# evandez/neuron-descriptions

Hardware: AMD Instinct MI355X
Metric: neuron-descriptions/sec (whole node), 4096 neurons x k=15 exemplars (higher is better)
Workload: dtype f32-equivalent: operands split into (hi,lo) f16 pairs (22 significant bits), 3 f16 MFMAs per product, f32 accumulate

## Files before the change

### neuron-descriptions_amd/csrc/common.h

```cpp
#pragma once
#include <hip/hip_runtime.h>
#include <stdint.h>
#include <stddef.h>
#include <string>
#include <vector>
#include <map>

#include "../../include/milan_hip.h"

#ifndef MILAN_EXPERIMENTS
#define MILAN_EXPERIMENTS 0
#endif

namespace milan {

void set_error(const char* fmt, ...);
#define MILAN_CHECK_HIP(expr)                                              \
  do {                                                                     \
    hipError_t _e = (expr);                                                \
    if (_e != hipSuccess) {                                                \
      milan::set_error("%s:%d: %s -> %s", __FILE__, __LINE__, #expr,       \
                       hipGetErrorString(_e));                             \
      return (int)_e;                                                      \
    }                                                                      \
// ... 54 lines not shown
  int chunk_major;
  float* C2;
  float* Cs;
  unsigned* status;
  int f16;
  const float* Wt;
  int tap_inner;
  const long long* lse_tgt;
  long lse_tgt_stride;
  float* lse_x;
  const int* m_live;
  const int* row_list;
  int m_live_mul;
  int tap_ncls;
  int tap_cls[MILAN_TAP_CLASSES][5];
};
static_assert(sizeof(GemmArgs) % 4 == 0, "GemmArgs is reloaded word by word");

enum OutMode : int { OUT_SCALAR = 0, OUT_VEC4 = 1, OUT_SPLIT8 = 2, OUT_F16 = 3 };

int launch_gemm(const GemmArgs& g, hipStream_t s);
bool row_list_supported(const GemmArgs& g);
void set_status_word(unsigned* word);
unsigned* status_word();
void profile_tag_kernel(int family);
int launch_zero_fill(void* p, size_t bytes, hipStream_t s);
int launch_f32_to_split(const float* src, long ld_src, float* dst, long ld_dst,
                        long rows, int K, float scale, hipStream_t s, int* nanrow = nullptr,
                        int stamp = 0);
int gemm_profile_enable(int enable);
int ensure_lds_attr(const void* kern, int bytes);
int device_cus8(int* out);
// ... 415 lines not shown
```

### neuron-descriptions_amd/csrc/decoder.hip

```cpp
#include "common.h"
#include <limits>
#include <optional>

namespace milan {

static constexpr float kFloatMin = -3.402823466e+38f;

static const Tensor* find(milan_ctx* c, const std::string& name) {
  auto it = c->raw.find(name);
  return it == c->raw.end() ? nullptr : &it->second;
}

__global__ void pack_rows_kernel(const float* __restrict__ src, int n, int k,
                                 int kp, float* __restrict__ dst) {
  const long total = (long)n * kp;
  for (long idx = blockIdx.x * (long)blockDim.x + threadIdx.x; idx < total;
       idx += (long)gridDim.x * blockDim.x) {
    const int r = idx / kp, col = idx - (long)r * kp;
    dst[idx] = col < k ? src[(long)r * k + col] : 0.f;
  }
}

__device__ inline int lstm_source_row(int i, int hidden) {
  if (!hidden) return i;
// ... 1722 lines not shown
  if (j < *live) out[j] = seqs[(long)urow[j] * L + col];
}

__global__ void lm_gather_rows_kernel(const float4* __restrict__ src, const int* __restrict__ idx,
                                      const int* __restrict__ live, int w4,
                                      float4* __restrict__ dst) {
  const long total = (long)*live * w4;
  for (long i = blockIdx.x * (long)blockDim.x + threadIdx.x; i < total;
       i += (long)gridDim.x * blockDim.x) {
    const long j = i / w4;
    const int q = (int)(i - j * w4);
    dst[i] = src[(long)idx[j] * w4 + q];
  }
}

struct LmDedup {
  int *cls, *urow, *par, *U;
  float *gh, *gc, *gv;
  int64_t *tok_c, *tgt_c;
};

static size_t lm_dedup_floats(const milan_dims& d, size_t R, int L, int G) {
  const size_t maps = 5 * (size_t)(L + 1) * R + 2 * (size_t)(L + 1) * G + (size_t)(L + 1) + 64;
  const size_t state = (2 * (size_t)d.lm_layers + 1) * R * d.lm_hidden_size;
  return maps + state + 4 * R + 2048;
}

static int lm_score_dedup(milan_ctx* c, const int64_t* seqs, int rows, int L, int group,
                          const int32_t* seq_len, int len_div, float* total, DecBuf* b,
                          float* scratch, hipStream_t s) {
// ... 11 lines not shown
  q.cls = (int*)take(sizeof(int) * (size_t)(L + 1) * R);
  q.urow = (int*)take(sizeof(int) * (size_t)(L + 1) * R);
  q.par = (int*)take(sizeof(int) * (size_t)(L + 1) * R);
  q.U = (int*)take(sizeof(int) * (size_t)(L + 1));
  q.gh = (float*)take(sizeof(float) * (size_t)d.lm_layers * R * Hl);
  q.gc = (float*)take(sizeof(float) * (size_t)d.lm_layers * R * Hl);
  q.gv = (float*)take(sizeof(float) * (size_t)R * Hl);
  q.tok_c = (int64_t*)take(sizeof(int64_t) * (size_t)R);
  q.tgt_c = (int64_t*)take(sizeof(int64_t) * (size_t)R);
  hipLaunchKernelGGL(lm_prefix_classes_kernel, dim3(G), dim3(256), 0, s, seqs, L, group, R, G,
                     rep, lrank, cnt);
  hipLaunchKernelGGL(lm_prefix_scan_kernel, dim3(L + 1), dim3(256), 0, s, cnt, G, offs, q.U);
  hipLaunchKernelGGL(lm_prefix_assign_kernel, dim3(nblk_all(R)), dim3(256), 0, s, rep, lrank, offs,
                     L, group, R, G, q.cls, q.urow, q.par);
  MILAN_CHECK_HIP(hipGetLastError());
  const size_t st_floats = (size_t)d.lm_layers * R * Hl;
  MILAN_TRY(launch_zero_fill(q.gh, sizeof(float) * st_floats, s));
  MILAN_TRY(launch_zero_fill(q.gc, sizeof(float) * st_floats, s));
  float* hs = b->lm_gates;
  float* emb_s = c->scratch;
  const size_t layer_sz = (size_t)R * Hl;
  int cur = 0;
  for (int t = 0; t + 1 < L; ++t) {
    const int p1 = t + 1, p2 = t + 2;
    const int* U1 = q.U + p1;
    const int* U2 = q.U + p2;
    LmState& st = b->lm[cur];
    LmState& nx = b->lm[cur ^ 1];
    hipLaunchKernelGGL(lm_gather_tok_kernel, dim3(nblk_all(R)), dim3(256), 0, s, seqs, (long)L, t,
                       q.urow + (size_t)p1 * R, U1, q.tok_c);
    hipLaunchKernelGGL(embed_split_kernel, dim3(nblk((long)R * (El / 8))), dim3(256), 0, s,
                       c->lm_embedding, q.tok_c, R, El, emb_s, El, c->emb_scale, status_word(),
                       U1);
    if (t > 0) {
      for (int l = 0; l < d.lm_layers; ++l) {
        hipLaunchKernelGGL(lm_gather_rows_kernel, dim3(nblk((long)R * (Hl / 4), 8192)), dim3(256),
// ... 48 lines not shown
    cur ^= 1;
  }
  MILAN_CHECK_HIP(hipGetLastError());
  return 0;
}

static int lm_score_impl(milan_ctx* c, const int64_t* seqs, int rows, int L,
                         const int32_t* seq_len, int len_div, float* total,
                         DecBuf* b, hipStream_t s, int group = 1,
                         float* dedup_scratch = nullptr, size_t dedup_floats = 0) {
  const milan_dims& d = c->d;
  MILAN_REQUIRE(d.has_lm && c->lm_out.w, MILAN_ERR_NO_LM,
                "cannot use MI/rerank decoding without an LM");
  const size_t st_bytes =
      sizeof(float) * (size_t)b->lm[0].rows * d.lm_hidden_size * d.lm_layers;
  MILAN_TRY(launch_zero_fill(b->lm[0].h, st_bytes, s));
  MILAN_TRY(launch_zero_fill(b->lm[0].c, st_bytes, s));
  if (L < 2) {
    MILAN_TRY(launch_zero_fill(total, sizeof(float) * rows, s));
    return 0;
  }
  int cur = 0;
  const bool split = lm_split_ok(c, rows) && (long)rows == b->lm[0].rows;
  static const bool lse_on = !(getenv("MILAN_LM_LSE") && atoi(getenv("MILAN_LM_LSE")) == 0);
  const bool lse = lse_on && d.vocab_size % 4 == 0 && d.vocab_size >= 256;
  if (split)
    MILAN_TRY(launch_zero_fill(b->lm_gates, sizeof(float) * (size_t)rows * d.lm_hidden_size * d.lm_layers, s));
  static const bool dedup_on = !(getenv("MILAN_LM_DEDUP") && atoi(getenv("MILAN_LM_DEDUP")) == 0);
  if (dedup_on && split && lse && group > 1 && group <= 256 && rows % group == 0 && dedup_scratch &&
      d.lm_hidden_size % 4 == 0 &&
      lm_dedup_floats(d, (size_t)rows, L, rows / group) <= dedup_floats)
    return lm_score_dedup(c, seqs, rows, L, group, seq_len, len_div, total, b, dedup_scratch, s);
  for (int t = 0; t + 1 < L; ++t) {
    hipLaunchKernelGGL(gather_col_kernel, dim3(nblk_all(rows)), dim3(256), 0, s, seqs,
                       (long)rows, (long)L, t, b->tok);
    if (split && lse) {
      const int nb = (d.vocab_size + 63) / 64;
      MILAN_TRY(lm_step_split(c, b->tok, rows, b->lm[cur], b->lm[cur ^ 1],
                              b->lm_gates, cur, b->lm_logits, s, seqs + t + 1, (long)L));
      hipLaunchKernelGGL(lm_accumulate_lse_kernel, dim3((rows + 3) / 4), dim3(256), 0, s,
                         b->lm_logits, nb, b->lm_logits + (size_t)rows * 2 * nb, rows, seqs,
                         (long)L, t, seq_len, len_div, d.stop_index, b->lm_alive, total);
      cur ^= 1;
      continue;
    }
    if (split)
      MILAN_TRY(lm_step_split(c, b->tok, rows, b->lm[cur], b->lm[cur ^ 1],
// ... 262 lines not shown
```

### neuron-descriptions_amd/csrc/encoder.hip

```cpp
#include "common.h"
#include <optional>
#include <vector>

#include <cstdlib>

namespace milan {

static constexpr float kBnEps = 1e-5f;

__global__ void pack_conv_kernel(const float* __restrict__ w, int cout, int cin,
                                 int cinp, int kh, int kw, int kp,
                                 const float* __restrict__ gamma,
                                 const float* __restrict__ beta,
                                 const float* __restrict__ mean,
                                 const float* __restrict__ var,
                                 float* __restrict__ wp,
                                 float* __restrict__ bias) {
  const long total = (long)cout * kp;
  for (long idx = blockIdx.x * (long)blockDim.x + threadIdx.x; idx < total;
       idx += (long)gridDim.x * blockDim.x) {
    const int o = idx / kp, k = idx - (long)o * kp;
    const int tap = k / cinp, i = k - tap * cinp;
    float v = 0.f;
    if (tap < kh * kw && i < cin) {
// ... 1034 lines not shown
  Levels lv;
  int h1, w1, hp, wp;
  float *in4, *raw, *x0, *x1, *ds, *t1, *t2;
  size_t x_sz, t1_sz, t2_sz;
  int *list_idx, *list_n;
  float* list_w;
  int* bbox;
  int* poison;
  int *order, *bbox_c, *count;
  int *tail_loc, *tail_cnt, *tail_off, *tail_rows, *tail_U;
  void* sh_hash;
  int *sh_rep, *sh_flag, *class_of;
  unsigned char* tail_s0;
  int *tail_loc3, *tail_cnt3, *tail_off3, *tail_rows3, *tail_U3;
  unsigned char* tail_s3;
};

static int conv_out(int h, int k, int s, int p) { return (h + 2 * p - k) / s + 1; }

static int plan(const milan_ctx* c, int n, int H, int W, Arena& a, EncPlan* pl) {
  const int wd = c->d.trunk_width;
  pl->h1 = conv_out(H, 7, 2, 3); pl->w1 = conv_out(W, 7, 2, 3);
  pl->hp = conv_out(pl->h1, 3, 2, 1); pl->wp = conv_out(pl->w1, 3, 2, 1);
  Levels& lv = pl->lv;
  lv.h[0] = pl->h1; lv.w[0] = pl->w1;
  lv.h[1] = pl->hp; lv.w[1] = pl->wp;
  for (int l = 2; l < 5; ++l) {
    lv.h[l] = conv_out(lv.h[l - 1], 3, 2, 1);
    lv.w[l] = conv_out(lv.w[l - 1], 3, 2, 1);
  }
// ... 33 lines not shown
    pl->tail_cnt = a.get<int>(3 * (size_t)n);
    pl->tail_off = a.get<int>(3 * (size_t)n);
    pl->tail_U = a.get<int>(4);
    pl->sh_hash = a.get<unsigned long long>((size_t)n);
    pl->sh_rep = a.get<int>((size_t)n);
    pl->sh_flag = a.get<int>((size_t)n);
    pl->class_of = a.get<int>((size_t)n);
    pl->tail_s0 = a.get<unsigned char>(((size_t)n * P4 + 3) & ~(size_t)3);
    const size_t P3 = (size_t)lv.h[3] * lv.w[3];
    pl->tail_loc3 = a.get<int>(2 * (size_t)n * P3);
    pl->tail_rows3 = a.get<int>(2 * (size_t)n * P3);
    pl->tail_cnt3 = a.get<int>(2 * (size_t)n);
    pl->tail_off3 = a.get<int>(2 * (size_t)n);
    pl->tail_U3 = a.get<int>(4);
    pl->tail_s3 = a.get<unsigned char>(((size_t)n * P3 + 3) & ~(size_t)3);
  }
  return 0;
}

static int encoder_sub_batch() {
  static int v = 0;
  if (v == 0) {
    const char* e = getenv("MILAN_ENC_SUB");
    v = e ? atoi(e) : 9600;
    if (v < 1) v = 9600;
  }
  return v;
}

static void alexnet_workspace_dry(const milan_ctx* c, int n, int H, int W,
// ... 437 lines not shown
    MILAN_TRY(lin(acol, 9 * P, b.c2, b.c2.wst, t2c, P, EPI_BIAS_RELU, nullptr, UO));
    hipLaunchKernelGGL(tail_rows_kernel<false>, dim3(blocks_for(rows_all * (Cin / 4))), dim3(256), 0, s,
                       (const float4*)X, rowsO, UO, Cin / 4, (float4*)rg);
    MILAN_TRY(lin(t2c, P, b.c3, b.c3.ws, yc, Cout, EPI_BIAS_RES_RELU, rg, UO));
    hipLaunchKernelGGL(tail_rows_kernel<true>, dim3(blocks_for(rows_all * (Cout / 4))), dim3(256), 0, s,
                       (const float4*)yc, rowsO, UO, Cout / 4, (float4*)Y);
    MILAN_CHECK_HIP(hipGetLastError());
    return 0;
  };

  auto on_list = [&](GemmArgs g, const int* rows, const int* U) {
    g.row_list = rows; g.m_live = U; g.m_live_mul = 1;
    return g;
  };
  auto list_ok = [&](const GemmArgs& g) { return row_list_supported(on_list(g, pl.tail_rows, pl.tail_U)); };
  auto tail_block_args = [&](const Bottleneck& b, const float* X, float* Y, float* T1, int hh,
                             int ww, GemmArgs* g1, GemmArgs* g2, GemmArgs* g3) {
    int h1, w1, h2, w2, h3, w3;
    *g1 = conv_args(b.c1, X, n, hh, ww, T1, EPI_BIAS_RELU, nullptr, c->zero, &h1, &w1, true);
    *g2 = conv_args(b.c2, T1, n, h1, w1, pl.t2, EPI_BIAS_RELU, nullptr, c->zero, &h2, &w2, true);
    *g3 = conv_args(b.c3, pl.t2, n, h2, w2, Y, EPI_BIAS_RES_RELU, X, c->zero, &h3, &w3, true);
  };
  auto tail_block_lists_ok = [&](const Bottleneck& b, int hh, int ww) {
    GemmArgs g1, g2, g3;
    tail_block_args(b, pl.x0, pl.x1, pl.t1, hh, ww, &g1, &g2, &g3);
    return lists && list_ok(g1) && list_ok(g2) && list_ok(g3);
  };
  auto tail_block_lists = [&](const Bottleneck& b, const float* X, float* Y, float* T1, int hh,
                              int ww, int kM, int kO) -> int {
    GemmArgs g1, g2, g3;
    tail_block_args(b, X, Y, T1, hh, ww, &g1, &g2, &g3);
    const int* rowsM = pl.tail_rows + (long)kM * n * P4;
    const int* rowsO = pl.tail_rows + (long)kO * n * P4;
    MILAN_TRY(launch_gemm(on_list(g1, rowsM, pl.tail_U + kM), s));
    MILAN_TRY(launch_gemm(on_list(g2, rowsO, pl.tail_U + kO), s));
    MILAN_TRY(launch_gemm(on_list(g3, rowsO, pl.tail_U + kO), s));
    return 0;
  };
  auto two_source_args = [&](const Bottleneck& b, const float* xin, float* yo, int hh, int ww,
                             int h2, int w2, int* h3, int* w3) {
    GemmArgs g3 = conv_args(b.c3d, pl.t2, n, h2, w2, yo, EPI_BIAS_RELU,
                            nullptr, c->zero, h3, w3, true);
    g3.Cin = b.c3.cin;
    g3.a_pix_stride = b.c3.cin;
    g3.a_img_stride = (long)h2 * w2 * b.c3.cin;
    g3.A2 = xin; g3.K1 = b.c3.K; g3.H2 = hh; g3.W2d = ww;
    g3.stride2 = b.down.stride;
    g3.a2_pix_stride = b.down.cin;
    g3.a2_img_stride = (long)hh * ww * b.down.cin;
    g3.flop_k = b.c3.K + b.down.K;
// ... 175 lines not shown
                   w2 == w && chain_supported(chain_P, b.down.cin, chain_NR);
      }
      const bool conv_front =
          (chain_plain || chain_ds) && (c->fusion & MILAN_FUSE_BNECK) && b.c2.K == b.c2.Kp &&
          b.c2.bias_s && conv3_p64_supported(b.c2.cin, b.c2.cout, b.c2.kh, b.c2.kw, b.c2.stride,
                                             b.c2.pad) &&
          chain_conv_supported(chain_P, chain_ds ? b.down.cin : 0, chain_NR, h1, w1);
      const bool c1_front =
          conv_front && c1_pending && chain_ds && b.c1.ws && b.c1.bias_s && b.c1.kh == 1 &&
          b.c1.kw == 1 && b.c1.stride == 1 && b.c1.cin == 64 && b.c1.cout == 64 &&
          b.c1.K == b.c1.Kp && h1 == h && w1 == w &&
          chain_conv_c1_supported(chain_P, b.down.cin, chain_NR, h1, w1);
      if (k0 >= 0 && li == 3 && bi == 0 && !chain_plain && !chain_ds && h == h3l && w == w3l) {
        const int* rows0 = pl.tail_rows + (long)k0 * n * P4;
        if (c1_pending) MILAN_TRY(launch_gemm(on_list(g1, rowsV, pl.tail_U3), s));
        MILAN_TRY(launch_gemm(on_list(g2, rows0, pl.tail_U + k0), s));
        GemmArgs g3 = two_source_args(b, x, y, h, w, h2, w2, &h3, &w3);
        MILAN_TRY(launch_gemm(on_list(g3, rows0, pl.tail_U + k0), s));
        float* tmp = x; x = y; y = tmp;
        h = h3; w = w3;
        continue;
      }
      if (lists_l3 && k0 >= 0 && li == 2 && last_of_stage && !chain_plain && !chain_ds &&
          h == h3l && w == w3l) {
        if (c1_pending) MILAN_TRY(gemm_t(g1));
        MILAN_TRY(launch_gemm(on_list(g2, rowsW, pl.tail_U3 + 1), s));
        GemmArgs g3 = conv_args(b.c3, pl.t2, n, h2, w2, y, EPI_BIAS_RES_RELU, x, c->zero, &h3, &w3, split);
        MILAN_TRY(launch_gemm(on_list(g3, rowsW, pl.tail_U3 + 1), s));
        float* tmp = x; x = y; y = tmp;
        h = h3; w = w3;
        continue;
      }
      if (c1_pending && !c1_front) MILAN_TRY(gemm_t(g1));
      if (conv_front) {
      } else if (split && (c->fusion & MILAN_FUSE_CONV3) && b.c2.K == b.c2.Kp &&
          conv3_p64_supported(b.c2.cin, b.c2.cout, b.c2.kh, b.c2.kw, b.c2.stride,
                              b.c2.pad)) {
        Conv3Args ca{};
        ca.in = t1buf; ca.ws = b.c2.ws; ca.bias = b.c2.bias_s; ca.acc_scale = b.c2.ws_inv;
        ca.out = pl.t2; ca.zero = c->zero; ca.n = n; ca.h = h1; ca.w = w1;
        ca.n_live = live;
// ... 378 lines not shown
```

### neuron-descriptions_amd/csrc/gemm.hip

```cpp
#include "common.h"

#include <map>
#include <mutex>
#include <utility>

#include <cstdio>
#include <cstdlib>
#include <cstring>
#include <type_traits>
#include <utility>
#include <vector>

#ifndef MILAN_ABLATE_BUILD
#define MILAN_ABLATE_BUILD 0
#endif
#ifndef MILAN_EXPERIMENTS
#define MILAN_EXPERIMENTS 0
#endif

namespace milan {

typedef float f32x16 __attribute__((ext_vector_type(16)));
typedef float f32x4 __attribute__((ext_vector_type(4)));
typedef _Float16 f16x8 __attribute__((ext_vector_type(8)));
// ... 1444 lines not shown

struct PpLoader {
  __amdgpu_buffer_rsrc_t srd_a, srd_a2, srd_w, cur_srd;
  unsigned row_off[4], row_off2[4], voff[4], vb[4];
  int hw0[4];
  unsigned mask[4];
  int ia, iw, is_kh, is_kw, is_cin0, seg_soff, cin_limit;
  unsigned a_bits, w_bits;
  int w_slice;
};

struct TapTile {
  int y0, ny, x0, nx;
  unsigned mask;
  int cnt, j, tile_n;
};

__device__ __forceinline__ bool tap_tile(const GemmArgs& g, int tiles_m, int tiles_n, TapTile* t) {
  const int b = blockIdx.x;
  if (g.tap_ncls == 0) {
    const int T = tiles_m * tiles_n;
    if (b >= T) return false;
    const int tile = xcd_tile(b, T);
    t->j = tile / tiles_n;
    t->tile_n = tile - t->j * tiles_n;
    t->y0 = 0; t->ny = g.Ho; t->x0 = 0; t->nx = g.Wo;
    t->mask = 0xffffffffu >> (32 - g.KH * g.KW);
    t->cnt = g.M;
    return true;
  }
// ... 6 lines not shown
    const int T = c < g.tap_ncls ? ((imgs * cw[c * 5 + 1] * cw[c * 5 + 3] + 255) >> 8) * tiles_n : 0;
    const int B = (T + 7) & ~7;
    if (cls < 0 && b < first + B) { cls = c; cfirst = first; ctiles = T; }
    first += B;
  }
  if (cls < 0) return false;
  const int bl = b - cfirst;
  if ((bl >> 3) >= (ctiles >> 3) + ((bl & 7) < (ctiles & 7))) return false;
  const int tile = xcd_tile(bl, ctiles);
  t->j = tile / tiles_n;
  t->tile_n = tile - t->j * tiles_n;
  t->y0 = cw[cls * 5]; t->ny = cw[cls * 5 + 1]; t->x0 = cw[cls * 5 + 2]; t->nx = cw[cls * 5 + 3];
  t->mask = (unsigned)cw[cls * 5 + 4];
  t->cnt = imgs * t->ny * t->nx;
  return true;
}

template <int BNW, bool F16 = false, bool TAPI = false, bool LIST = false>
__device__ __forceinline__ void split16_pp32_tile(int tile_m, int tile_n, int tid, bool prefetched,
                                                  bool has_next, int ntile_m, int ntile_n,
                                                  TapTile tt = TapTile{}) {
  const GemmArgs g = reload_gemm_args();
  constexpr int BM = 256, BN = 256, BKP = 32, TM = BNW == 256 ? 4 : 2, TN = 2;
  static_assert(BNW == 256 || BNW == 128, "ping-pong tile: 256 or 128 columns");
  constexpr int SLOTF = BM * BKP;
  constexpr unsigned OOB = 0x80000000u;
  extern __shared__ __attribute__((aligned(16))) float smem[];
  auto a_slot = [&](int sl) { return smem + (sl < 2 ? sl : 3) * SLOTF; };
  auto w_slot = [&](int sl) { return smem + (sl == 0 ? 2 : 4) * SLOTF; };
  const int lane = tid & 63;
// ... 36 lines not shown
    else x = rem0 + (ok ? row : 0);
    int dimg = (int)((float)x * r_howo);
    dimg -= (dimg * pix_img > x);
    dimg += ((dimg + 1) * pix_img <= x);
    const int rem = x - dimg * pix_img;
    int ho = (int)((float)rem * r_wo);
    ho -= (ho * pix_row > rem);
    ho += ((ho + 1) * pix_row <= rem);
    *dimg_out = dimg;
    *wo_out = rem - ho * pix_row + (TAPI ? tt.x0 : 0);
    *ho_out = ho + (TAPI ? tt.y0 : 0);
    return ok;
  };
  auto setup = [&](PpLoader& L, int tm, int tn) {
    const int prow = lane >> 3, pos = lane & 7;
    const int m0 = tm * BM;
    const int img0 = LIST ? list_slot0(m0) : m0 / pix_img;
    const int rem0 = LIST ? img0 * pix_img : m0 - img0 * pix_img;
    const long bias = ((long)g.pad * g.Wd + g.pad) * g.a_pix_stride;
    L.srd_a = __builtin_amdgcn_make_buffer_rsrc(
        const_cast<float*>(g.A + (long)img0 * g.a_img_stride - bias), 0, 0x7fffffff, 0x00020000);
    L.srd_a2 = __builtin_amdgcn_make_buffer_rsrc(
        const_cast<float*>(g.A2 ? g.A2 + (long)img0 * g.a2_img_stride : g.A), 0, 0x7fffffff,
        0x00020000);
    L.srd_w = __builtin_amdgcn_make_buffer_rsrc(const_cast<float*>(g.W + (long)tn * BNW * g.Kp), 0,
                                                0x7fffffff, 0x00020000);
#pragma unroll
    for (int it = 0; it < 4; ++it) {
      const int row = it * 64 + wave * 8 + prow;
      const int q = pos ^ ((row >> 1) & 7);
      int dimg, ho, wo;
// ... 256 lines not shown
  __builtin_amdgcn_s_barrier();
  if (has_next) {
    PpLoader N;
    setup(N, ntile_m, ntile_n);
    issue_a(N, I0{}, true);
    issue_w(N, I0{}, true);
    issue_a(N, I1{}, true);
  }
  const GemmArgs ge = reload_gemm_args<LIST>();
#pragma unroll
  for (int i = 0; i < TM; ++i)
#pragma unroll
    for (int j = 0; j < TN; ++j) acc[i][j] = acc[i][j] * ge.acc_scale;
  if constexpr (LIST) {
    int* tab = reinterpret_cast<int*>(a_slot(0)) + wave * (TM * 32);
    const int m0 = tile_m * BM;
#pragma unroll
    for (int e = 0; e < TM * 32 / 64; ++e) {
      const int r = e * 64 + lane;
      const int m = m0 + wm * (TM * 32) + r;
      tab[r] = m < rows_all ? ge.row_list[m] : 0x7fffffff;
    }
    run_epilogue<TM, TN, true, true>(ge, acc, a_slot(2), wave, lane, 0, tile_n * BNW + wn * 64, tab);
  } else if constexpr (TAPI) {
    int* tab = reinterpret_cast<int*>(a_slot(0)) + wave * (TM * 32);
    const int m0 = tile_m * BM;
    const int img0 = m0 / pix_img;
    const int rem0 = m0 - img0 * pix_img;
#pragma unroll
    for (int e = 0; e < TM * 32 / 64; ++e) {
      const int r = e * 64 + lane;
// ... 53 lines not shown
template <int BNW>
__global__ __launch_bounds__(512, 2) void igemm_split16_pp32t_kernel(GemmArgs g, int tiles_m,
                                                                     int tiles_n) {
  tiles_m = live_tiles_m(g, tiles_m, 256);
  TapTile tt;
  if (!tap_tile(g, tiles_m, tiles_n, &tt)) return;
  int tid = threadIdx.x;
  asm volatile("" : "+v"(tid));
  split16_pp32_tile<BNW, false, true>(tt.j, tt.tile_n, tid, false, false, tt.j, tt.tile_n, tt);
}

template <bool TAPI>
__global__ __launch_bounds__(512, 2) void igemm_split16_pp32l_kernel(GemmArgs g, int tiles_m,
                                                                     int tiles_n) {
  tiles_m = live_tiles_m(g, tiles_m, 256);
  const int T = tiles_m * tiles_n;
  const int q = blockIdx.x;
  if (q >= T) return;
  const int tile = xcd_tile(q, T);
  const int tile_m = tile / tiles_n, tile_n = tile - tile_m * tiles_n;
  TapTile tt{};
  if constexpr (TAPI) {
    tt.ny = g.Ho; tt.nx = g.Wo;
    tt.mask = 0xffffffffu >> (32 - g.KH * g.KW);
    tt.cnt = g.M;
  }
  int tid = threadIdx.x;
  asm volatile("" : "+v"(tid));
  split16_pp32_tile<256, false, TAPI, true>(tile_m, tile_n, tid, false, false, tile_m, tile_n, tt);
}

template <int BNW, bool TAPI>
__global__ __launch_bounds__(512, 2) void igemm_f16_pp32_kernel(GemmArgs g, int tiles_m, int tiles_n) {
  tiles_m = live_tiles_m(g, tiles_m, 256);
  if constexpr (TAPI) {
    TapTile tt;
    if (!tap_tile(g, tiles_m, tiles_n, &tt)) return;
    int tid = threadIdx.x;
    asm volatile("" : "+v"(tid));
    split16_pp32_tile<BNW, true, true>(tt.j, tt.tile_n, tid, false, false, tt.j, tt.tile_n, tt);
// ... 500 lines not shown
  auto kern = igemm_split16_tm2_kernel<BM, BN, STAGES>;
  MILAN_TRY(ensure_lds_attr(reinterpret_cast<const void*>(kern), (int)lds));
  hipLaunchKernelGGL(kern, dim3(tiles_m * tiles_n), dim3(NT), lds, s, g, tiles_m,
                     tiles_n);
  MILAN_CHECK_HIP(hipGetLastError());
  return 0;
}

static bool tap_inner_wanted(const GemmArgs& g) {
  static int on = -1;
  if (on < 0) { const char* e = getenv("MILAN_TAP_INNER"); on = e ? atoi(e) : 1; }
  return on && g.Wt && !g.A2 && g.KH * g.KW > 1 && g.KH * g.KW <= 32 && g.K == g.Kp &&
         g.Cin % 32 == 0;
}

static int tap_classes(GemmArgs& t, int tiles_m, int tiles_n) {
  static int on = -1;
  if (on < 0) { const char* e = getenv("MILAN_TAP_SKIP"); on = e ? atoi(e) : 1; }
  const bool wanted = on && t.tap_ncls >= 0;
  t.tap_ncls = 0;
  const int howo = t.Ho * t.Wo;
  if (!wanted || howo <= 0 || t.M % howo != 0 || (t.m_live && t.m_live_mul % howo != 0))
    return tiles_m * tiles_n;
  struct Run { int o0, n; unsigned set; };
  auto runs = [](int size, int out, int k, int stride, int pad, Run* r) {
    int n = 0;
    for (int o = 0; o < out; ++o) {
      unsigned set = 0;
      for (int i = 0; i < k; ++i)
        if (o * stride - pad + i >= 0 && o * stride - pad + i < size) set |= 1u << i;
      if (n > 0 && r[n - 1].set == set) { ++r[n - 1].n; continue; }
      if (n == MILAN_TAP_CLASSES) return MILAN_TAP_CLASSES + 1;
      r[n++] = Run{o, 1, set};
    }
    return n;
  };
  Run ry[MILAN_TAP_CLASSES], rx[MILAN_TAP_CLASSES];
  const int nry = runs(t.H, t.Ho, t.KH, t.stride, t.pad, ry);
  const int nrx = runs(t.Wd, t.Wo, t.KW, t.stride, t.pad, rx);
  if (nry * nrx > MILAN_TAP_CLASSES) return tiles_m * tiles_n;
  int cls[MILAN_TAP_CLASSES][5], n = 0, min_pix = howo;
  for (int a = 0; a < nry; ++a)
    for (int b = 0; b < nrx; ++b, ++n) {
      unsigned mask = 0;
      for (int kh = 0; kh < t.KH; ++kh)
        for (int kw = 0; kw < t.KW; ++kw)
          if ((ry[a].set >> kh & 1u) && (rx[b].set >> kw & 1u)) mask |= 1u << (kh * t.KW + kw);
      if (mask == 0) return tiles_m * tiles_n;
      const int c[5] = {ry[a].o0, ry[a].n, rx[b].o0, rx[b].n, (int)mask};
      int at = n;
      while (at > 0 && __builtin_popcount((unsigned)cls[at - 1][4]) < __builtin_popcount(mask)) {
        memcpy(cls[at], cls[at - 1], sizeof(c));
        --at;
      }
      memcpy(cls[at], c, sizeof(c));
      if (ry[a].n * rx[b].n < min_pix) min_pix = ry[a].n * rx[b].n;
    }
  if ((256L / min_pix + 2) * t.a_img_stride * 4 + 64 >= 0x7fffffffL) return tiles_m * tiles_n;
  const long imgs = t.M / howo;
  long grid = 0;
  for (int c = 0; c < n; ++c)
    grid += ((imgs * cls[c][1] * cls[c][3] + 255) / 256 * tiles_n + 7) / 8 * 8;
  if (grid >= 0x7fffffffL) return tiles_m * tiles_n;
  t.tap_ncls = n;
  memcpy(t.tap_cls, cls, sizeof(int) * 5 * n);
  return (int)grid;
}

static thread_local bool t_row_list_taken = false;

template <int BNW>
static int launch_split16_pp32(const GemmArgs& g, hipStream_t s) {
  const int tiles_m = (g.M + 255) / 256, tiles_n = (g.N + BNW - 1) / BNW;
  const size_t lds = size_t(5) * 256 * 32 * sizeof(float);
  if (g.row_list != nullptr) {
    if (BNW != 256) return MILAN_ERR_SHAPE;
    t_row_list_taken = true;
    GemmArgs t = g;
    const bool tapi = tap_inner_wanted(g);
    if (tapi) { t.W = g.Wt; t.tap_inner = 1; }
    t.tap_ncls = 0;
    profile_tag_kernel(tapi ? MILAN_KERNEL_PP32T_256 : MILAN_KERNEL_PP32_256);
    auto kern = tapi ? igemm_split16_pp32l_kernel<true> : igemm_split16_pp32l_kernel<false>;
    MILAN_TRY(ensure_lds_attr(reinterpret_cast<const void*>(kern), (int)lds));
    hipLaunchKernelGGL(kern, dim3(tiles_m * tiles_n), dim3(512), lds, s, t, tiles_m, tiles_n);
    MILAN_CHECK_HIP(hipGetLastError());
    return 0;
  }
  if (tap_inner_wanted(g)) {
    GemmArgs t = g;
    t.W = g.Wt;
    t.tap_inner = 1;
    const int grid = tap_classes(t, tiles_m, tiles_n);
    profile_tag_kernel(BNW == 256 ? MILAN_KERNEL_PP32T_256 : MILAN_KERNEL_PP32_128);
    auto kern = igemm_split16_pp32t_kernel<BNW>;
    MILAN_TRY(ensure_lds_attr(reinterpret_cast<const void*>(kern), (int)lds));
    hipLaunchKernelGGL(kern, dim3(grid), dim3(512), lds, s, t, tiles_m, tiles_n);
    MILAN_CHECK_HIP(hipGetLastError());
    return 0;
  }
// ... 169 lines not shown
bool row_list_supported(const GemmArgs& g) {
  static int pp = -1;
  if (pp < 0) { const char* e = getenv("MILAN_PP"); pp = e ? atoi(e) : 1; }
  const long howo = (long)g.Ho * g.Wo;
  if (g.row_list == nullptr || g.m_live == nullptr || g.m_live_mul != 1) return false;
  if (!g.a_split || g.f16 || g.chunk_major || g.aniso || g.tile_hint != 0 || env_tile_hint() != 0 ||
      env_tile_override(g.N, g.K) != 0 || pp != 1)
    return false;
#if MILAN_EXPERIMENTS
  if (conv3x3_enabled() || (getenv("MILAN_SCHED") && atoi(getenv("MILAN_SCHED")))) return false;
#endif
  if (g.epilogue == EPI_LSE || g.epilogue == EPI_LSTM || !g.out_split) return false;
  if (g.N % 256 != 0 || g.Cin % 32 != 0 || g.K != g.Kp || !pp_eligible(g)) return false;
  if (g.A2 && (g.K1 % 32 != 0 || g.KH != 1 || g.KW != 1)) return false;
  if (g.KH * g.KW > 1 && !tap_inner_wanted(g)) return false;
  if ((long)g.H + g.pad >= 32768 || (long)g.Wd + g.pad >= 32768) return false;
  if (howo <= 0 || g.M % howo != 0 || 257 * howo >= (1L << 24)) return false;
  if (258 * g.a_img_stride * 4 + 64 >= 0x7fffffffL) return false;
  if (g.A2 && 258 * g.a2_img_stride * 4 + 64 >= 0x7fffffffL) return false;
  return true;
}

static int launch_gemm_impl(GemmArgs g, hipStream_t s) {
  const bool cin32 = (g.Cin % 32 == 0);
  if (g.status == nullptr) g.status = status_word();
  if (g.tile_hint == 0) g.tile_hint = env_tile_hint();
  if (const int o = env_tile_override(g.N, g.K)) g.tile_hint = o;
  {
    static int dbg = -1;
    if (dbg < 0) { const char* e = getenv("MILAN_ABLATE"); dbg = e ? atoi(e) : 0; }
// ... 160 lines not shown
```

Baseline: 1439.

## Sort row-list 3x3 conv rows by tap class to skip padded taps

Adds count, scan and fill kernels that regroup the sparse row list of the tail-stage 3x3 convolutions by border tap class. The row-list GEMM kernel then walks per-class segments and applies each class's tap mask, so it skips padded taps for border pixels. The LM dedup path now runs before the full-state zero fills, and a row-limited zero kernel replaces its own full zero fills. The cost is three extra small launches per sorted GEMM, more grid tiles with partial-tile waste per segment, and a serial segment search at the start of each block.

```diff
diff --git a/neuron-descriptions_amd/csrc/common.h b/neuron-descriptions_amd/csrc/common.h
--- a/neuron-descriptions_amd/csrc/common.h
+++ b/neuron-descriptions_amd/csrc/common.h
@@ -92,8 +92,29 @@
   int m_live_mul;
   int tap_ncls;
   int tap_cls[MILAN_TAP_CLASSES][5];
+  const int* list_seg;
+  int list_nseg;
 };
 static_assert(sizeof(GemmArgs) % 4 == 0, "GemmArgs is reloaded word by word");
+
+constexpr int MILAN_LIST_SEGS = 36;
+struct RowListClasses {
+  int ncls, blk_slots, nblk;
+  int cls[MILAN_TAP_CLASSES][5];
+};
+bool row_list_classes(const GemmArgs& g, RowListClasses* rc);
+inline size_t row_list_sort_ints(size_t n) { return 2 * n * MILAN_TAP_CLASSES; }
+int launch_row_list_sort(const RowListClasses& rc, const int* loc, const int* cnt, int n, int P,
+                         int Wo, int* scratch, int* seg, int* rows, hipStream_t s);
+inline GemmArgs on_sorted_list(GemmArgs g, const RowListClasses& rc, const int* rows,
+                               const int* seg, const int* live) {
+  g.row_list = rows; g.m_live = live; g.m_live_mul = 1;
+  g.list_seg = seg; g.list_nseg = rc.nblk * rc.ncls;
+  g.tap_ncls = rc.ncls;
+  for (int c = 0; c < rc.ncls; ++c)
+    for (int i = 0; i < 5; ++i) g.tap_cls[c][i] = rc.cls[c][i];
+  return g;
+}
 
 enum OutMode : int { OUT_SCALAR = 0, OUT_VEC4 = 1, OUT_SPLIT8 = 2, OUT_F16 = 3 };
 
diff --git a/neuron-descriptions_amd/csrc/decoder.hip b/neuron-descriptions_amd/csrc/decoder.hip
--- a/neuron-descriptions_amd/csrc/decoder.hip
+++ b/neuron-descriptions_amd/csrc/decoder.hip
@@ -1760,6 +1760,18 @@
   }
 }
 
+__global__ void lm_zero_rows_kernel(const int* __restrict__ live, int w4, int layers, long layer4,
+                                    float4* __restrict__ a, float4* __restrict__ b) {
+  const long total = (long)*live * w4;
+  const float4 z = make_float4(0.f, 0.f, 0.f, 0.f);
+  for (long i = blockIdx.x * (long)blockDim.x + threadIdx.x; i < total;
+       i += (long)gridDim.x * blockDim.x)
+    for (int l = 0; l < layers; ++l) {
+      a[l * layer4 + i] = z;
+      b[l * layer4 + i] = z;
+    }
+}
+
 struct LmDedup {
   int *cls, *urow, *par, *U;
   float *gh, *gc, *gv;
@@ -1801,12 +1813,12 @@
   hipLaunchKernelGGL(lm_prefix_assign_kernel, dim3(nblk_all(R)), dim3(256), 0, s, rep, lrank, offs,
                      L, group, R, G, q.cls, q.urow, q.par);
   MILAN_CHECK_HIP(hipGetLastError());
-  const size_t st_floats = (size_t)d.lm_layers * R * Hl;
-  MILAN_TRY(launch_zero_fill(q.gh, sizeof(float) * st_floats, s));
-  MILAN_TRY(launch_zero_fill(q.gc, sizeof(float) * st_floats, s));
   float* hs = b->lm_gates;
   float* emb_s = c->scratch;
   const size_t layer_sz = (size_t)R * Hl;
+  hipLaunchKernelGGL(lm_zero_rows_kernel, dim3(nblk((long)R * (Hl / 4), 8192)), dim3(256), 0, s,
+                     q.U + 1, Hl / 4, d.lm_layers, (long)(layer_sz / 4), (float4*)q.gh,
+                     (float4*)q.gc);
   int cur = 0;
   for (int t = 0; t + 1 < L; ++t) {
     const int p1 = t + 1, p2 = t + 2;
@@ -1885,6 +1897,14 @@
                 "cannot use MI/rerank decoding without an LM");
   const size_t st_bytes =
       sizeof(float) * (size_t)b->lm[0].rows * d.lm_hidden_size * d.lm_layers;
+  const bool split = lm_split_ok(c, rows) && (long)rows == b->lm[0].rows;
+  static const bool lse_on = !(getenv("MILAN_LM_LSE") && atoi(getenv("MILAN_LM_LSE")) == 0);
+  const bool lse = lse_on && d.vocab_size % 4 == 0 && d.vocab_size >= 256;
+  static const bool dedup_on = !(getenv("MILAN_LM_DEDUP") && atoi(getenv("MILAN_LM_DEDUP")) == 0);
+  if (L >= 2 && dedup_on && split && lse && group > 1 && group <= 256 && rows % group == 0 &&
+      dedup_scratch && d.lm_hidden_size % 4 == 0 &&
+      lm_dedup_floats(d, (size_t)rows, L, rows / group) <= dedup_floats)
+    return lm_score_dedup(c, seqs, rows, L, group, seq_len, len_div, total, b, dedup_scratch, s);
   MILAN_TRY(launch_zero_fill(b->lm[0].h, st_bytes, s));
   MILAN_TRY(launch_zero_fill(b->lm[0].c, st_bytes, s));
   if (L < 2) {
@@ -1892,16 +1912,8 @@
     return 0;
   }
   int cur = 0;
-  const bool split = lm_split_ok(c, rows) && (long)rows == b->lm[0].rows;
-  static const bool lse_on = !(getenv("MILAN_LM_LSE") && atoi(getenv("MILAN_LM_LSE")) == 0);
-  const bool lse = lse_on && d.vocab_size % 4 == 0 && d.vocab_size >= 256;
   if (split)
     MILAN_TRY(launch_zero_fill(b->lm_gates, sizeof(float) * (size_t)rows * d.lm_hidden_size * d.lm_layers, s));
-  static const bool dedup_on = !(getenv("MILAN_LM_DEDUP") && atoi(getenv("MILAN_LM_DEDUP")) == 0);
-  if (dedup_on && split && lse && group > 1 && group <= 256 && rows % group == 0 && dedup_scratch &&
-      d.lm_hidden_size % 4 == 0 &&
-      lm_dedup_floats(d, (size_t)rows, L, rows / group) <= dedup_floats)
-    return lm_score_dedup(c, seqs, rows, L, group, seq_len, len_div, total, b, dedup_scratch, s);
   for (int t = 0; t + 1 < L; ++t) {
     hipLaunchKernelGGL(gather_col_kernel, dim3(nblk_all(rows)), dim3(256), 0, s, seqs,
                        (long)rows, (long)L, t, b->tok);
diff --git a/neuron-descriptions_amd/csrc/encoder.hip b/neuron-descriptions_amd/csrc/encoder.hip
--- a/neuron-descriptions_amd/csrc/encoder.hip
+++ b/neuron-descriptions_amd/csrc/encoder.hip
@@ -1072,6 +1072,7 @@
   unsigned char* tail_s0;
   int *tail_loc3, *tail_cnt3, *tail_off3, *tail_rows3, *tail_U3;
   unsigned char* tail_s3;
+  int *tail_cls_rows, *tail_cls_scr, *tail_cls_seg;
 };
 
 static int conv_out(int h, int k, int s, int p) { return (h + 2 * p - k) / s + 1; }
@@ -1135,6 +1136,9 @@
     pl->tail_off3 = a.get<int>(2 * (size_t)n);
     pl->tail_U3 = a.get<int>(4);
     pl->tail_s3 = a.get<unsigned char>(((size_t)n * P3 + 3) & ~(size_t)3);
+    pl->tail_cls_rows = a.get<int>((size_t)n * (P3 > P4 ? P3 : P4));
+    pl->tail_cls_scr = a.get<int>(row_list_sort_ints((size_t)n));
+    pl->tail_cls_seg = a.get<int>(MILAN_LIST_SEGS);
   }
   return 0;
 }
@@ -1602,6 +1606,19 @@
     return g;
   };
   auto list_ok = [&](const GemmArgs& g) { return row_list_supported(on_list(g, pl.tail_rows, pl.tail_U)); };
+  auto launch_list_taps = [&](const GemmArgs& g, const int* rows, const int* U, const int* loc,
+                              const int* cnt) -> int {
+    RowListClasses rc;
+    if (row_list_classes(g, &rc)) {
+      const GemmArgs t = on_sorted_list(g, rc, pl.tail_cls_rows, pl.tail_cls_seg, U);
+      if (row_list_supported(t)) {
+        MILAN_TRY(launch_row_list_sort(rc, loc, cnt, n, g.Ho * g.Wo, g.Wo, pl.tail_cls_scr,
+                                       pl.tail_cls_seg, pl.tail_cls_rows, s));
+        return launch_gemm(t, s);
+      }
+    }
+    return launch_gemm(on_list(g, rows, U), s);
+  };
   auto tail_block_args = [&](const Bottleneck& b, const float* X, float* Y, float* T1, int hh,
                              int ww, GemmArgs* g1, GemmArgs* g2, GemmArgs* g3) {
     int h1, w1, h2, w2, h3, w3;
@@ -1621,7 +1638,11 @@
     const int* rowsM = pl.tail_rows + (long)kM * n * P4;
     const int* rowsO = pl.tail_rows + (long)kO * n * P4;
     MILAN_TRY(launch_gemm(on_list(g1, rowsM, pl.tail_U + kM), s));
-    MILAN_TRY(launch_gemm(on_list(g2, rowsO, pl.tail_U + kO), s));
+    if (kO > 0)
+      MILAN_TRY(launch_list_taps(g2, rowsO, pl.tail_U + kO, pl.tail_loc + (long)kO * n * P4,
+                                 pl.tail_cnt + (long)kO * n));
+    else
+      MILAN_TRY(launch_gemm(on_list(g2, rowsO, pl.tail_U + kO), s));
     MILAN_TRY(launch_gemm(on_list(g3, rowsO, pl.tail_U + kO), s));
     return 0;
   };
@@ -1827,7 +1848,8 @@
       if (k0 >= 0 && li == 3 && bi == 0 && !chain_plain && !chain_ds && h == h3l && w == w3l) {
         const int* rows0 = pl.tail_rows + (long)k0 * n * P4;
         if (c1_pending) MILAN_TRY(launch_gemm(on_list(g1, rowsV, pl.tail_U3), s));
-        MILAN_TRY(launch_gemm(on_list(g2, rows0, pl.tail_U + k0), s));
+        MILAN_TRY(launch_list_taps(g2, rows0, pl.tail_U + k0, pl.tail_loc + (long)k0 * n * P4,
+                                   pl.tail_cnt + (long)k0 * n));
         GemmArgs g3 = two_source_args(b, x, y, h, w, h2, w2, &h3, &w3);
         MILAN_TRY(launch_gemm(on_list(g3, rows0, pl.tail_U + k0), s));
         float* tmp = x; x = y; y = tmp;
@@ -1837,7 +1859,8 @@
       if (lists_l3 && k0 >= 0 && li == 2 && last_of_stage && !chain_plain && !chain_ds &&
           h == h3l && w == w3l) {
         if (c1_pending) MILAN_TRY(gemm_t(g1));
-        MILAN_TRY(launch_gemm(on_list(g2, rowsW, pl.tail_U3 + 1), s));
+        MILAN_TRY(launch_list_taps(g2, rowsW, pl.tail_U3 + 1, pl.tail_loc3 + (long)n * P3,
+                                   pl.tail_cnt3 + n));
         GemmArgs g3 = conv_args(b.c3, pl.t2, n, h2, w2, y, EPI_BIAS_RES_RELU, x, c->zero, &h3, &w3, split);
         MILAN_TRY(launch_gemm(on_list(g3, rowsW, pl.tail_U3 + 1), s));
         float* tmp = x; x = y; y = tmp;
diff --git a/neuron-descriptions_amd/csrc/gemm.hip b/neuron-descriptions_amd/csrc/gemm.hip
--- a/neuron-descriptions_amd/csrc/gemm.hip
+++ b/neuron-descriptions_amd/csrc/gemm.hip
@@ -1482,6 +1482,7 @@
   int y0, ny, x0, nx;
   unsigned mask;
   int cnt, j, tile_n;
+  int base;
 };
 
 __device__ __forceinline__ bool tap_tile(const GemmArgs& g, int tiles_m, int tiles_n, TapTile* t) {
@@ -1518,6 +1519,34 @@
   t->mask = (unsigned)cw[cls * 5 + 4];
   t->cnt = imgs * t->ny * t->nx;
   return true;
+}
+
+__device__ __forceinline__ bool list_tile(const GemmArgs& g, int tiles_n, TapTile* t) {
+  typedef const int __attribute__((address_space(4)))* KArgWords;
+  const KArgWords cw = (KArgWords)__builtin_amdgcn_kernarg_segment_ptr() + offsetof(GemmArgs, tap_cls) / 4;
+  const int b = blockIdx.x;
+  int first = 0, base = 0;
+  for (int s = 0; s < g.list_nseg; ++s) {
+    const int rows = g.list_seg[s];
+    const int T = ((rows + 255) >> 8) * tiles_n;
+    const int B = (T + 7) & ~7;
+    if (b < first + B) {
+      const int bl = b - first;
+      if ((bl >> 3) >= (T >> 3) + ((bl & 7) < (T & 7))) return false;
+      const int tile = xcd_tile(bl, T);
+      const int cls = s % g.tap_ncls;
+      t->j = tile / tiles_n;
+      t->tile_n = tile - t->j * tiles_n;
+      t->y0 = 0; t->ny = g.Ho; t->x0 = 0; t->nx = g.Wo;
+      t->mask = (unsigned)cw[cls * 5 + 4];
+      t->base = base;
+      t->cnt = base + rows;
+      return true;
+    }
+    first += B;
+    base += rows;
+  }
+  return false;
 }
 
 template <int BNW, bool F16 = false, bool TAPI = false, bool LIST = false>
@@ -1584,7 +1613,7 @@
   };
   auto setup = [&](PpLoader& L, int tm, int tn) {
     const int prow = lane >> 3, pos = lane & 7;
-    const int m0 = tm * BM;
+    const int m0 = tm * BM + (LIST && TAPI ? tt.base : 0);
     const int img0 = LIST ? list_slot0(m0) : m0 / pix_img;
     const int rem0 = LIST ? img0 * pix_img : m0 - img0 * pix_img;
     const long bias = ((long)g.pad * g.Wd + g.pad) * g.a_pix_stride;
@@ -1871,7 +1900,7 @@
     for (int j = 0; j < TN; ++j) acc[i][j] = acc[i][j] * ge.acc_scale;
   if constexpr (LIST) {
     int* tab = reinterpret_cast<int*>(a_slot(0)) + wave * (TM * 32);
-    const int m0 = tile_m * BM;
+    const int m0 = tile_m * BM + (TAPI ? tt.base : 0);
 #pragma unroll
     for (int e = 0; e < TM * 32 / 64; ++e) {
       const int r = e * 64 + lane;
@@ -1955,16 +1984,22 @@
 __global__ __launch_bounds__(512, 2) void igemm_split16_pp32l_kernel(GemmArgs g, int tiles_m,
                                                                      int tiles_n) {
   tiles_m = live_tiles_m(g, tiles_m, 256);
-  const int T = tiles_m * tiles_n;
-  const int q = blockIdx.x;
-  if (q >= T) return;
-  const int tile = xcd_tile(q, T);
-  const int tile_m = tile / tiles_n, tile_n = tile - tile_m * tiles_n;
   TapTile tt{};
-  if constexpr (TAPI) {
-    tt.ny = g.Ho; tt.nx = g.Wo;
-    tt.mask = 0xffffffffu >> (32 - g.KH * g.KW);
-    tt.cnt = g.M;
+  int tile_m, tile_n;
+  if (TAPI && g.list_nseg > 0) {
+    if (!list_tile(g, tiles_n, &tt)) return;
+    tile_m = tt.j; tile_n = tt.tile_n;
+  } else {
+    const int T = tiles_m * tiles_n;
+    const int q = blockIdx.x;
+    if (q >= T) return;
+    const int tile = xcd_tile(q, T);
+    tile_m = tile / tiles_n; tile_n = tile - tile_m * tiles_n;
+    if constexpr (TAPI) {
+      tt.ny = g.Ho; tt.nx = g.Wo;
+      tt.mask = 0xffffffffu >> (32 - g.KH * g.KW);
+      tt.cnt = g.M;
+    }
   }
   int tid = threadIdx.x;
   asm volatile("" : "+v"(tid));
@@ -2495,14 +2530,14 @@
          g.Cin % 32 == 0;
 }
 
-static int tap_classes(GemmArgs& t, int tiles_m, int tiles_n) {
+static bool tap_skip_on() {
   static int on = -1;
   if (on < 0) { const char* e = getenv("MILAN_TAP_SKIP"); on = e ? atoi(e) : 1; }
-  const bool wanted = on && t.tap_ncls >= 0;
-  t.tap_ncls = 0;
+  return on != 0;
+}
+
+static int tap_class_table(const GemmArgs& t, int (*cls)[5], int* min_pix_out) {
   const int howo = t.Ho * t.Wo;
-  if (!wanted || howo <= 0 || t.M % howo != 0 || (t.m_live && t.m_live_mul % howo != 0))
-    return tiles_m * tiles_n;
   struct Run { int o0, n; unsigned set; };
   auto runs = [](int size, int out, int k, int stride, int pad, Run* r) {
     int n = 0;
@@ -2519,15 +2554,15 @@
   Run ry[MILAN_TAP_CLASSES], rx[MILAN_TAP_CLASSES];
   const int nry = runs(t.H, t.Ho, t.KH, t.stride, t.pad, ry);
   const int nrx = runs(t.Wd, t.Wo, t.KW, t.stride, t.pad, rx);
-  if (nry * nrx > MILAN_TAP_CLASSES) return tiles_m * tiles_n;
-  int cls[MILAN_TAP_CLASSES][5], n = 0, min_pix = howo;
+  if (nry * nrx > MILAN_TAP_CLASSES) return 0;
+  int n = 0, min_pix = howo;
   for (int a = 0; a < nry; ++a)
     for (int b = 0; b < nrx; ++b, ++n) {
       unsigned mask = 0;
       for (int kh = 0; kh < t.KH; ++kh)
         for (int kw = 0; kw < t.KW; ++kw)
           if ((ry[a].set >> kh & 1u) && (rx[b].set >> kw & 1u)) mask |= 1u << (kh * t.KW + kw);
-      if (mask == 0) return tiles_m * tiles_n;
+      if (mask == 0) return 0;
       const int c[5] = {ry[a].o0, ry[a].n, rx[b].o0, rx[b].n, (int)mask};
       int at = n;
       while (at > 0 && __builtin_popcount((unsigned)cls[at - 1][4]) < __builtin_popcount(mask)) {
@@ -2537,6 +2572,19 @@
       memcpy(cls[at], c, sizeof(c));
       if (ry[a].n * rx[b].n < min_pix) min_pix = ry[a].n * rx[b].n;
     }
+  *min_pix_out = min_pix;
+  return n;
+}
+
+static int tap_classes(GemmArgs& t, int tiles_m, int tiles_n) {
+  const bool wanted = tap_skip_on() && t.tap_ncls >= 0;
+  t.tap_ncls = 0;
+  const int howo = t.Ho * t.Wo;
+  if (!wanted || howo <= 0 || t.M % howo != 0 || (t.m_live && t.m_live_mul % howo != 0))
+    return tiles_m * tiles_n;
+  int cls[MILAN_TAP_CLASSES][5], min_pix = howo;
+  const int n = tap_class_table(t, cls, &min_pix);
+  if (n == 0) return tiles_m * tiles_n;
   if ((256L / min_pix + 2) * t.a_img_stride * 4 + 64 >= 0x7fffffffL) return tiles_m * tiles_n;
   const long imgs = t.M / howo;
   long grid = 0;
@@ -2546,6 +2594,147 @@
   t.tap_ncls = n;
   memcpy(t.tap_cls, cls, sizeof(int) * 5 * n);
   return (int)grid;
+}
+
+bool row_list_classes(const GemmArgs& g, RowListClasses* rc) {
+  rc->ncls = rc->blk_slots = rc->nblk = 0;
+  const long howo = (long)g.Ho * g.Wo;
+  if (!tap_skip_on() || g.tap_ncls < 0 || !tap_inner_wanted(g) || howo <= 0 || g.M % howo != 0 ||
+      g.a_img_stride <= 0)
+    return false;
+  int min_pix = 0;
+  const int n = tap_class_table(g, rc->cls, &min_pix);
+  const unsigned all = 0xffffffffu >> (32 - g.KH * g.KW);
+  if (n == 0 || (n == 1 && (unsigned)rc->cls[0][4] == all)) return false;
+  const long slots = g.M / howo;
+  long reach = (0x7fffffffL - 64) / (g.a_img_stride * 4) - 2;
+  const long exact = ((1L << 24) - 1) / howo - 1;
+  if (exact < reach) reach = exact;
+  if (reach < 1) return false;
+  const long nblk = (slots + reach - 1) / reach;
+  if (nblk * n > MILAN_LIST_SEGS) return false;
+  rc->ncls = n;
+  rc->nblk = (int)nblk;
+  rc->blk_slots = (int)((slots + nblk - 1) / nblk);
+  return true;
+}
+
+struct ListClsTab { int ncls, c[MILAN_TAP_CLASSES][4]; };
+
+__device__ __forceinline__ int list_pixel_class(const ListClsTab& t, int p, int Wo) {
+  const int y = p / Wo, x = p - y * Wo;
+  int r = 0;
+#pragma unroll
+  for (int c = 0; c < MILAN_TAP_CLASSES; ++c)
+    if (c < t.ncls && y >= t.c[c][0] && y < t.c[c][0] + t.c[c][1] && x >= t.c[c][2] &&
+        x < t.c[c][2] + t.c[c][3])
+      r = c;
+  return r;
+}
+
+__global__ __launch_bounds__(64) void list_class_count_kernel(ListClsTab t, const int* __restrict__ loc,
+                                                              const int* __restrict__ cnt, int P, int Wo,
+                                                              int* __restrict__ slot_cnt) {
+  const int j = blockIdx.x, lane = threadIdx.x;
+  const int c = cnt[j];
+  int mine[MILAN_TAP_CLASSES];
+#pragma unroll
+  for (int k = 0; k < MILAN_TAP_CLASSES; ++k) mine[k] = 0;
+  for (int i0 = 0; i0 < c; i0 += 64) {
+    const int i = i0 + lane;
+    const int k = i < c ? list_pixel_class(t, loc[(long)j * P + i], Wo) : -1;
+#pragma unroll
+    for (int q = 0; q < MILAN_TAP_CLASSES; ++q) mine[q] += __popcll(__ballot(k == q));
+  }
+  if (lane == 0) {
+#pragma unroll
+    for (int q = 0; q < MILAN_TAP_CLASSES; ++q)
+      if (q < t.ncls) slot_cnt[(long)j * t.ncls + q] = mine[q];
+  }
+}
+
+__global__ __launch_bounds__(256) void list_class_scan_kernel(const int* __restrict__ slot_cnt, int n,
+                                                              int ncls, int blk_slots,
+                                                              int* __restrict__ slot_off,
+                                                              int* __restrict__ seg) {
+  __shared__ int tmp[256];
+  const int s = blockIdx.x, tid = threadIdx.x;
+  const int blk = s / ncls, c = s - blk * ncls;
+  const int j_lo = blk * blk_slots, j_hi = min(n, j_lo + blk_slots);
+  const int per = (j_hi - j_lo + 255) / 256;
+  const int a = min(j_hi, j_lo + tid * per), b = min(j_hi, a + per);
+  int sum = 0;
+  for (int j = a; j < b; ++j) sum += slot_cnt[(long)j * ncls + c];
+  tmp[tid] = sum;
+  __syncthreads();
+  for (int o = 1; o < 256; o <<= 1) {
+    const int add = tid >= o ? tmp[tid - o] : 0;
+    __syncthreads();
+    tmp[tid] += add;
+    __syncthreads();
+  }
+  int run = tmp[tid] - sum;
+  for (int j = a; j < b; ++j) {
+    slot_off[(long)j * ncls + c] = run;
+    run += slot_cnt[(long)j * ncls + c];
+  }
+  if (tid == 255) seg[s] = tmp[255];
+}
+
+__global__ __launch_bounds__(64) void list_class_fill_kernel(ListClsTab t, const int* __restrict__ loc,
+                                                             const int* __restrict__ cnt, int P, int Wo,
+                                                             int blk_slots,
+                                                             const int* __restrict__ slot_off,
+                                                             const int* __restrict__ seg,
+                                                             int* __restrict__ rows) {
+  __shared__ int s_base[MILAN_TAP_CLASSES];
+  const int j = blockIdx.x, lane = threadIdx.x;
+  const int c = cnt[j];
+  if (c == 0) return;
+  if (lane < t.ncls) {
+    const int s = (j / blk_slots) * t.ncls + lane;
+    int b = slot_off[(long)j * t.ncls + lane];
+    for (int q = 0; q < s; ++q) b += seg[q];
+    s_base[lane] = b;
+  }
+  __syncthreads();
+  int run[MILAN_TAP_CLASSES];
+#pragma unroll
+  for (int k = 0; k < MILAN_TAP_CLASSES; ++k) run[k] = 0;
+  for (int i0 = 0; i0 < c; i0 += 64) {
+    const int i = i0 + lane;
+    const int p = i < c ? loc[(long)j * P + i] : 0;
+    const int k = i < c ? list_pixel_class(t, p, Wo) : -1;
+    int pos = -1;
+#pragma unroll
+    for (int q = 0; q < MILAN_TAP_CLASSES; ++q) {
+      const unsigned long long m = __ballot(k == q);
+      if (k == q) pos = s_base[q] + run[q] + __popcll(m & ((1ull << lane) - 1ull));
+      run[q] += __popcll(m);
+    }
+    if (pos >= 0) rows[pos] = j * P + p;
+  }
+}
+
+int launch_row_list_sort(const RowListClasses& rc, const int* loc, const int* cnt, int n, int P,
+                         int Wo, int* scratch, int* seg, int* rows, hipStream_t s) {
+  MILAN_REQUIRE(rc.ncls >= 1 && rc.ncls <= MILAN_TAP_CLASSES && rc.nblk >= 1 && rc.blk_slots >= 1 &&
+                    rc.nblk * rc.ncls <= MILAN_LIST_SEGS && (long)rc.nblk * rc.blk_slots >= n && n > 0,
+                MILAN_ERR_ARG, "row list sort: bad class plan (%d classes, %d x %d slots, n=%d)",
+                rc.ncls, rc.nblk, rc.blk_slots, n);
+  ListClsTab t{};
+  t.ncls = rc.ncls;
+  for (int c = 0; c < rc.ncls; ++c)
+    for (int i = 0; i < 4; ++i) t.c[c][i] = rc.cls[c][i];
+  int* slot_cnt = scratch;
+  int* slot_off = scratch + (size_t)n * MILAN_TAP_CLASSES;
+  hipLaunchKernelGGL(list_class_count_kernel, dim3(n), dim3(64), 0, s, t, loc, cnt, P, Wo, slot_cnt);
+  hipLaunchKernelGGL(list_class_scan_kernel, dim3(rc.nblk * rc.ncls), dim3(256), 0, s, slot_cnt, n,
+                     rc.ncls, rc.blk_slots, slot_off, seg);
+  hipLaunchKernelGGL(list_class_fill_kernel, dim3(n), dim3(64), 0, s, t, loc, cnt, P, Wo,
+                     rc.blk_slots, slot_off, seg, rows);
+  MILAN_CHECK_HIP(hipGetLastError());
+  return 0;
 }
 
 static thread_local bool t_row_list_taken = false;
@@ -2560,11 +2749,18 @@
     GemmArgs t = g;
     const bool tapi = tap_inner_wanted(g);
     if (tapi) { t.W = g.Wt; t.tap_inner = 1; }
-    t.tap_ncls = 0;
+    long grid = (long)tiles_m * tiles_n;
+    if (tapi && g.list_nseg > 0) {
+      grid = ((long)tiles_m + g.list_nseg) * tiles_n + 7L * g.list_nseg;
+      if (grid >= 0x7fffffffL) return MILAN_ERR_SHAPE;
+    } else {
+      t.tap_ncls = 0;
+      t.list_nseg = 0;
+    }
     profile_tag_kernel(tapi ? MILAN_KERNEL_PP32T_256 : MILAN_KERNEL_PP32_256);
     auto kern = tapi ? igemm_split16_pp32l_kernel<true> : igemm_split16_pp32l_kernel<false>;
     MILAN_TRY(ensure_lds_attr(reinterpret_cast<const void*>(kern), (int)lds));
-    hipLaunchKernelGGL(kern, dim3(tiles_m * tiles_n), dim3(512), lds, s, t, tiles_m, tiles_n);
+    hipLaunchKernelGGL(kern, dim3((int)grid), dim3(512), lds, s, t, tiles_m, tiles_n);
     MILAN_CHECK_HIP(hipGetLastError());
     return 0;
   }
@@ -2764,6 +2960,10 @@
   if (g.N % 256 != 0 || g.Cin % 32 != 0 || g.K != g.Kp || !pp_eligible(g)) return false;
   if (g.A2 && (g.K1 % 32 != 0 || g.KH != 1 || g.KW != 1)) return false;
   if (g.KH * g.KW > 1 && !tap_inner_wanted(g)) return false;
+  if (g.list_nseg != 0 &&
+      (g.list_nseg < 0 || g.list_nseg > MILAN_LIST_SEGS || g.list_seg == nullptr || g.tap_ncls < 1 ||
+       g.tap_ncls > MILAN_TAP_CLASSES || g.list_nseg % g.tap_ncls != 0 || g.KH * g.KW <= 1))
+    return false;
   if ((long)g.H + g.pad >= 32768 || (long)g.Wd + g.pad >= 32768) return false;
   if (howo <= 0 || g.M % howo != 0 || 257 * howo >= (1L << 24)) return false;
   if (258 * g.a_img_stride * 4 + 64 >= 0x7fffffffL) return false;
```

After: 1436. About the same (-0.2%).
